# myrrix/myrrix-recommender

Measured on AMD Instinct MI355X. Metric: ALS rows solved/sec (full iteration) at k=64, higher is better.
Workload: dtype f32 storage; per-row Gramian: f16x2-split operands (22 bits), f32 accumulate; Cholesky f32

## Files before the change

myrrix-recommender_amd/csrc/als_kernels.h:

```cpp
#pragma once
#include <hip/hip_runtime.h>
#include <stdint.h>

#include <type_traits>

namespace mals {

#ifndef MALS_WAVES
#define MALS_WAVES(T, MODE) ((T) <= 4 ? 4 : ((T) == 5 ? 3 : 2))
#endif
#ifndef MALS_WAVES_H
#define MALS_WAVES_H(T, MODE) ((T) <= 2 ? 5 : ((T) <= 4 ? 3 : 2))
#endif

typedef float f32x4 __attribute__((ext_vector_type(4)));
typedef double f64x4 __attribute__((ext_vector_type(4)));

__host__ __device__ constexpr int tri(int T) { return T * (T + 1) / 2; }
__host__ __device__ constexpr int tidx(int T, int i, int j) { return i * T - (i * (i - 1)) / 2 + (j - i); }

constexpr int YMAX_SLOTS = 64;

struct WorkItem {
  int64_t begin;
// ... 1638 lines not shown
  }
  if (Gf) {
    const float f = (row < k && col < k) ? (float)s : 0.f;
    const int lr = row - 16 * i, lc = col - 16 * j;
    Gf[(t * 64 + 16 * (lr >> 2) + lc) * 4 + (lr & 3)] = f;
    if (i == j) Gf[(t * 64 + 16 * (lc >> 2) + lr) * 4 + (lc & 3)] = f;
  }
}

__global__ void gramian_ref_latch_kernel(int* state) { state[3] = (state[0] != 0 && state[1] == 0) ? 1 : 0; }

template <int T>
__global__ __launch_bounds__(256) void gramian_ref_kernel(const float* __restrict__ M, int64_t n_rows, int k, int* state,
                                                          double* __restrict__ part, double* __restrict__ Gref) {
  if (state[3] == 0) return;
  constexpr int KP = 16 * T, NE = T * T;
  __shared__ float srow[8][KP];
  __shared__ int s_last;
  const int tid = threadIdx.x;
  double acc[NE];
#pragma unroll
  for (int j = 0; j < NE; ++j) acc[j] = 0.0;
  const int64_t per = (n_rows + gridDim.x - 1) / gridDim.x;
  const int64_t r0 = per * blockIdx.x, r1 = r0 + per < n_rows ? r0 + per : n_rows;
  for (int64_t base = r0; base < r1; base += 8) {
    __syncthreads();
    for (int e = tid; e < 8 * KP; e += 256) {
      const int i = e / KP, f = e - i * KP;
      srow[i][f] = (base + i < r1 && f < k) ? M[(base + i) * k + f] : 0.f;
    }
    __syncthreads();
#pragma unroll
    for (int i = 0; i < 8; ++i) {
#pragma unroll
      for (int j = 0; j < NE; ++j) {
        const int e = tid + 256 * j, r = e / KP, c = e - r * KP;
        acc[j] += (double)__fmul_rn(srow[i][r], srow[i][c]);
      }
    }
  }
#pragma unroll
  for (int j = 0; j < NE; ++j) part[(size_t)blockIdx.x * (KP * KP) + tid + 256 * j] = acc[j];
  __threadfence();
  __syncthreads();
  if (tid == 0) s_last = atomicAdd(&state[2], 1) == (int)gridDim.x - 1;
  __syncthreads();
  if (!s_last) return;
  __threadfence();
#pragma unroll
  for (int j = 0; j < NE; ++j) {
    const int e = tid + 256 * j, r = e / KP, c = e - r * KP;
    double sum = 0.0;
    for (unsigned w = 0; w < gridDim.x; ++w) sum += part[(size_t)w * (KP * KP) + e];
    if (r < k && c < k) Gref[(int64_t)r * k + c] = sum;
  }
  __threadfence();
  __syncthreads();
  if (tid == 0) {
    state[2] = 0;
    state[1] = 1;
  }
}

template <int T>
__global__ __launch_bounds__(256, 2) void gramian_split_kernel(const float* __restrict__ M, int64_t n_rows, int k,
                                                               int64_t rows_per_slab, float* __restrict__ partial,
                                                               unsigned* __restrict__ ymax) {
  constexpr int E = T <= 4 ? 8 : 4, STEP = 4 * E;
  const int lane = threadIdx.x & 63, g = lane >> 4, c = lane & 15;
  const int64_t slab = uniform64((int64_t)blockIdx.x * 4 + (threadIdx.x >> 6));
  const int64_t r0 = slab * rows_per_slab;
  int64_t r1 = r0 + rows_per_slab;
  if (r1 > n_rows) r1 = n_rows;
  f32x4 acc[tri(T)];
#pragma unroll
  for (int t = 0; t < tri(T); ++t) acc[t] = f32x4{0.f, 0.f, 0.f, 0.f};
  int pw = 100;
  int slab_max = 0;
  const int n_slab = (int)(r1 - r0);
  const float* __restrict__ base = M + (n_slab > 0 ? r0 : 0) * k;
  const bool kfull = k == 16 * T;
  int fo[T];
#pragma unroll
  for (int v = 0; v < T; ++v) fo[v] = 16 * v + c < k ? 16 * v + c : k - 1;
  auto load_step = [&](int rl, float (&raw)[T][E]) {
    if (rl + STEP <= n_slab) {
      const char* bb = reinterpret_cast<const char*>(base);
      const unsigned o0 = 4u * (unsigned)((rl + E * g) * k + c), last = 4u * (unsigned)(fo[T - 1] - c);
      if (kfull) {
#pragma unroll
        for (int s4 = 0; s4 < E; ++s4) {
          const unsigned o = o0 + 4u * (unsigned)(s4 * k);
#pragma unroll
          for (int v = 0; v < T; ++v) raw[v][s4] = *reinterpret_cast<const float*>(bb + o + 64 * v);
        }
      } else {
#pragma unroll
        for (int s4 = 0; s4 < E; ++s4) {
          const unsigned o = o0 + 4u * (unsigned)(s4 * k);
#pragma unroll
          for (int v = 0; v < T - 1; ++v) raw[v][s4] = *reinterpret_cast<const float*>(bb + o + 64 * v);
          raw[T - 1][s4] = *reinterpret_cast<const float*>(bb + (o + last));
        }
      }
    } else {
#pragma unroll
      for (int s4 = 0; s4 < E; ++s4) {
        const int row = rl + E * g + s4;
        const unsigned o = (unsigned)((row < n_slab ? row : 0) * k);
#pragma unroll
        for (int v = 0; v < T; ++v) raw[v][s4] = base[o + (unsigned)fo[v]];
      }
    }
  };
  auto do_step = [&](int rl, float (&raw)[T][E], int reload) {
    if (rl + STEP > n_slab) {
#pragma unroll
      for (int s4 = 0; s4 < E; ++s4)
        if (!(rl + E * g + s4 < n_slab))
#pragma unroll
          for (int v = 0; v < T; ++v) raw[v][s4] = 0.f;
    }
    if (!kfull) {
      if (!(16 * (T - 1) + c < k))
#pragma unroll
        for (int s4 = 0; s4 < E; ++s4) raw[T - 1][s4] = 0.f;
    }
    float amax = 0.f;
#pragma unroll
    for (int s4 = 0; s4 < E; ++s4)
#pragma unroll
      for (int v = 0; v < T; ++v) amax = fmaxf(amax, fabsf(raw[v][s4]));
    int m = __float_as_int(amax);
    for (int off = 32; off > 0; off >>= 1) m = max(m, __shfl_xor(m, off));
    m = uniform(m);
    slab_max = max(slab_max, m);
    if (m != 0) {
      const int eb = ((m >> 23) & 255) - 126;
      const int want = 14 - eb;
      if (want < pw) {
        if (pw != 100) {
          int d2 = 2 * (want - pw);
          d2 = d2 < -120 ? -120 : d2;
          const float f = __int_as_float((d2 + 127) << 23);
#pragma unroll
          for (int t = 0; t < tri(T); ++t) acc[t] *= f;
        }
        pw = want;
      }
    }
    const int pwc = pw == 100 ? 0 : (pw < -100 ? -100 : (pw > 100 ? 100 : pw));
    const float sc = __int_as_float((pwc + 127) << 23);
    ZOp<E> zh[T], zl[T];
#pragma unroll
    for (int v = 0; v < T; ++v) {
#pragma unroll
      for (int pr = 0; pr < E / 2; ++pr) {
        const float z0 = raw[v][2 * pr] * sc, z1 = raw[v][2 * pr + 1] * sc;
        const int h01 = pk_rn16(z0, z1);
        zh[v].r[pr] = h01;
        zl[v].r[pr] = pk_rn16(residual_lo(h01, z0), residual_hi(h01, z1));
      }
    }
    __builtin_amdgcn_sched_barrier(0);
    load_step(reload, raw);
    __builtin_amdgcn_sched_barrier(0);
#pragma unroll
    for (int i = 0; i < T; ++i)
#pragma unroll
      for (int j = i; j < T; ++j) acc[tidx(T, i, j)] = mfma_h<E>(zh[i], zh[j], acc[tidx(T, i, j)]);
#pragma unroll
    for (int i = 0; i < T; ++i)
#pragma unroll
      for (int j = i; j < T; ++j) acc[tidx(T, i, j)] = mfma_h<E>(zh[i], zl[j], acc[tidx(T, i, j)]);
#pragma unroll
    for (int i = 0; i < T; ++i)
#pragma unroll
      for (int j = i; j < T; ++j) acc[tidx(T, i, j)] = mfma_h<E>(zl[i], zh[j], acc[tidx(T, i, j)]);
  };
  if constexpr (T <= 6) {
    float ra[T][E], rb[T][E];
    load_step(0, ra);
    load_step(STEP, rb);
    for (int rl = 0; rl < n_slab; rl += 2 * STEP) {
      do_step(rl, ra, rl + 2 * STEP);
      do_step(rl + STEP, rb, rl + 3 * STEP);
    }
  } else {
    float ra[T][E];
    load_step(0, ra);
    for (int rl = 0; rl < n_slab; rl += STEP) do_step(rl, ra, rl + STEP);
  }
  int d2 = pw == 100 ? 0 : -2 * pw;
  d2 = d2 < -126 ? -126 : (d2 > 126 ? 126 : d2);
  const float back = __int_as_float((d2 + 127) << 23);
  float* o = partial + slab * (int64_t)(tri(T) * 4 * 64) + lane;
#pragma unroll
  for (int t = 0; t < tri(T); ++t)
#pragma unroll
    for (int r = 0; r < 4; ++r) o[(t * 4 + r) * 64] = acc[t][r] * back;
  if (ymax) {
    __shared__ int s_max[4];
    if (lane == 0) s_max[threadIdx.x >> 6] = slab_max;
    __syncthreads();
    if (threadIdx.x == 0) {
      const unsigned m4 = (unsigned)max(max(s_max[0], s_max[1]), max(s_max[2], s_max[3]));
      unsigned* slot = ymax + (blockIdx.x & (YMAX_SLOTS - 1));
      if (m4 > __builtin_nontemporal_load(slot)) atomicMax(slot, m4);
    }
  }
}

__global__ void gramian_pack_kernel(const double* __restrict__ G, int k, int T, float* __restrict__ Gf) {
  const int e = blockIdx.x * blockDim.x + threadIdx.x;
  if (e >= tri(T) * 256) return;
  const int t = e >> 8, lane = (e >> 2) & 63, reg = e & 3;
  int i = 0, rem = t;
  while (rem >= T - i) {
    rem -= T - i;
    ++i;
  }
  const int j = i + rem;
  const int row = 16 * i + 4 * (lane >> 4) + reg, col = 16 * j + (lane & 15);
  Gf[e] = (row < k && col < k) ? (float)G[(int64_t)row * k + col] : 0.f;
}

__global__ void gather_scale_kernel(const double* __restrict__ G, int k, float sqrt_w_max, float sqrt_w_mean, double n_rows,
                                    int force_flag, const unsigned* __restrict__ ymax, float* __restrict__ out) {
  if (blockIdx.x != 0 || threadIdx.x >= 64) return;
  const int lane = threadIdx.x;
  double d = 0.0, tr = 0.0;
  for (int f = lane; f < k; f += 64) {
    const double g = G[(int64_t)f * k + f];
    d = fmax(d, g);
    tr += g;
  }
  unsigned bits = (ymax && lane < YMAX_SLOTS) ? ymax[lane] : 0u;
  static_assert(YMAX_SLOTS <= 64, "one slot per lane");
  for (int off = 32; off > 0; off >>= 1) {
    d = fmax(d, __shfl_xor(d, off));
    tr += __shfl_xor(tr, off);
    bits = max(bits, (unsigned)__shfl_xor((int)bits, off));
  }
  if (lane != 0) return;
  double ybound = sqrt(d);
  if (ymax) {
    const float ym = __uint_as_float(bits);
    if (ym > 0.f && ym < 3.0e38f && (double)ym < ybound) ybound = (double)ym;
  }
  out[3] = (float)ybound;
  const double bound = ybound * (double)sqrt_w_max;
  int e = 0;
  if (bound > 0.0 && bound < 1.0e300) {
    int eb;
    (void)frexp(bound, &eb);
    e = 14 - eb;
    e = e < -60 ? -60 : (e > 60 ? 60 : e);
  }
  out[0] = (float)ldexp(1.0, e);
  out[1] = (float)ldexp(1.0, -2 * e);
  const double typical = (double)sqrt_w_mean * sqrt(tr / ((double)k * fmax(n_rows, 1.0)));
  float ok = 1.f;
  if (typical > 0.0 && bound > 0.0 && bound / typical > 65536.0) ok = 0.f;
  if (!(bound < 1.0e300)) ok = 0.f;
  if (force_flag >= 0) ok = (float)force_flag;
  out[2] = ok;
}

__global__ void max_abs_kernel(const float* __restrict__ v, int64_t n, unsigned* __restrict__ out, double* __restrict__ sum_out) {
  float m = 0.f;
  double s = 0.0;
  for (int64_t i = (int64_t)blockIdx.x * blockDim.x + threadIdx.x; i < n; i += (int64_t)gridDim.x * blockDim.x) {
    const float a = fabsf(v[i]);
    m = fmaxf(m, a);
    s += (double)a;
  }
  for (int off = 32; off > 0; off >>= 1) {
    m = fmaxf(m, __shfl_xor(m, off));
    s += __shfl_xor(s, off);
  }
  if ((threadIdx.x & 63) == 0) {
    atomicMax(out, __float_as_uint(m));
    atomicAdd(sum_out, s);
  }
}

__global__ void col_range_kernel(const int32_t* __restrict__ col, int64_t n, int* __restrict__ out) {
  int lo = 0x7fffffff, hi = (int)0x80000000;
  for (int64_t i = (int64_t)blockIdx.x * blockDim.x + threadIdx.x; i < n; i += (int64_t)gridDim.x * blockDim.x) {
    const int c = col[i];
    lo = min(lo, c);
    hi = max(hi, c);
  }
  for (int off = 32; off > 0; off >>= 1) {
    lo = min(lo, __shfl_xor(lo, off));
    hi = max(hi, __shfl_xor(hi, off));
  }
  if ((threadIdx.x & 63) == 0) {
    atomicMin(out, lo);
    atomicMax(out + 1, hi);
  }
}

template <int T>
__global__ __launch_bounds__(256) void reconstruction_kernel(const int64_t* __restrict__ row_ptr, const int32_t* __restrict__ col,
                                                             const float* __restrict__ X, const float* __restrict__ Y, int k,
                                                             int64_t n_rows, double* __restrict__ partial_sum,
                                                             unsigned long long* __restrict__ partial_cnt) {
  const int lane = threadIdx.x & 63, g = lane >> 4, c = lane & 15;
  const int64_t wave = (int64_t)blockIdx.x * 4 + (threadIdx.x >> 6), n_waves = (int64_t)gridDim.x * 4;
  double acc = 0.0;
  unsigned long long cnt = 0;
  for (int64_t row = wave; row < n_rows; row += n_waves) {
    const int64_t b = row_ptr[row], e = row_ptr[row + 1];
    float x[T];
#pragma unroll
    for (int v = 0; v < T; ++v) x[v] = 16 * v + c < k ? X[row * k + 16 * v + c] : 0.f;
    for (int64_t s = b; s < e; s += 4) {
      const bool ok = s + g < e;
      const float* y = Y + (int64_t)col[ok ? s + g : b] * k;
      double d = 0.0;
#pragma unroll
      for (int v = 0; v < T; ++v) {
        const float yv = 16 * v + c < k ? y[16 * v + c] : 0.f;
        d += (double)__fmul_rn(x[v], yv);
      }
#pragma unroll
      for (int off = 8; off > 0; off >>= 1) d += __shfl_xor(d, off);
      if (ok && c == 0) {
        acc += fmax(0.0, 1.0 - d);
        ++cnt;
      }
    }
  }
  acc += __shfl_xor(acc, 16);
  acc += __shfl_xor(acc, 32);
  cnt += __shfl_xor(cnt, 16);
  cnt += __shfl_xor(cnt, 32);
  if (lane == 0) {
    partial_sum[wave] = acc;
    partial_cnt[wave] = cnt;
  }
}

__global__ void sample_dots_kernel(const float* __restrict__ X, const float* __restrict__ Y, const int64_t* __restrict__ users,
                                   const int64_t* __restrict__ items, int n_users, int n_items, int k, double* __restrict__ out) {
  const int e = blockIdx.x * blockDim.x + threadIdx.x;
  if (e >= n_users * n_items) return;
  const float* x = X + users[e / n_items] * (int64_t)k;
  const float* y = Y + items[e % n_items] * (int64_t)k;
  double d = 0.0;
  for (int f = 0; f < k; ++f) d += (double)__fmul_rn(x[f], y[f]);
  out[e] = d;
}

__global__ void pad_rows_kernel(const float* __restrict__ src, int64_t n, int k, int ld, float* __restrict__ dst) {
  const int q = ld >> 2;
  const int64_t n4 = n * q;
  for (int64_t e = (int64_t)blockIdx.x * blockDim.x + threadIdx.x; e < n4; e += (int64_t)gridDim.x * blockDim.x) {
    const int64_t r = e / q;
    const int f = 4 * (int)(e - r * q);
    const float* s = src + r * k + f;
    f32x4 v;
#pragma unroll
    for (int i = 0; i < 4; ++i) v[i] = f + i < k ? s[i] : 0.f;
    reinterpret_cast<f32x4*>(dst)[e] = v;
  }
}

__global__ void gather_rows_kernel(const float* __restrict__ F, const int64_t* __restrict__ idx, int n, int k,
                                   float* __restrict__ out) {
  const int e = blockIdx.x * blockDim.x + threadIdx.x;
  if (e >= n * k) return;
  out[e] = F[idx[e / k] * (int64_t)k + (e % k)];
}

}
```

myrrix-recommender_amd/csrc/mals_api.hip:

```cpp
#include "../../include/myrrix_als.h"
#include "als_kernels.h"
#include "dual_kernels.h"
#include "lds_kernels.h"
#include "host_eigen.h"
#include "host_solver.h"
#include "topn_kernels.h"
#include "mals_internal.h"
#include "hip_buffer.h"

#include <hip/hip_runtime.h>

#include <algorithm>
#include <atomic>
#include <chrono>
#include <cmath>
#include <cstdio>
#include <cstdlib>
#include <condition_variable>
#include <cstring>
#include <deque>
#include <limits>
#include <mutex>
#include <new>
#include <string>
#include <thread>
#include <type_traits>
#include <vector>

#ifndef MALS_D4
#define MALS_D4 4
#endif
using namespace mals;

namespace {

struct SideState {
  int64_t n_total = 0;
  float* F = nullptr;
  DeviceBuffer<float> F_own;
  int64_t row_offset = 0, n_local = 0, nnz = 0;
  int64_t* row_ptr = nullptr;
  int32_t* col = nullptr;
  float* val = nullptr;
  DeviceBuffer<int64_t> row_ptr_own;
  DeviceBuffer<int32_t> col_own;
  DeviceBuffer<float> val_own;
  bool has_matrix = false;
  std::vector<int64_t> h_row_ptr;
  int64_t append_rows = 0, append_nnz = 0;
  bool appending = false;
  DeviceBuffer<WorkItem> itemsA;
  int64_t nA = 0;
  int64_t nnzA = 0, nnzB = 0;
  DeviceBuffer<WorkItem> itemsB;
  int64_t nB = 0;
  DeviceBuffer<RowC> rowsC;
  int64_t nC = 0;
  DeviceBuffer<float> scratch;
  DeviceBuffer<uint8_t> refine;
  int32_t col_min = 0, col_max = -1;
  float max_abs_val = 0.f;
  float local_max_abs_val = 0.f;
  double mean_abs_val = 0.0;
  double local_mean_abs_val = 0.0;
  struct ChunkRange {
    int64_t offA = 0, nA = 0, nnzA = 0, offB = 0, nB = 0, nnzB = 0, offC = 0, nC = 0;
    int64_t offP = 0, nP = 0;
    int64_t nD[4] = {0, 0, 0, 0}, nnzD[4] = {0, 0, 0, 0}, nZ = 0;
    int64_t n_dual() const { return nD[0] + nD[1] + nD[2] + nD[3]; }
    int64_t nnz_dual() const { return nnzD[0] + nnzD[1] + nnzD[2] + nnzD[3]; }
  };
  int64_t n_dual_rows = 0;
  int64_t chunk_rows_override = -1;
  std::vector<ChunkRange> chunks;
  DeviceBuffer<double> G;
  DeviceBuffer<float> Gf;
  DeviceBuffer<uint8_t> partials;
  bool G_valid = false;
  uint64_t G_version = 0;
  DeviceBuffer<unsigned> d_ymax;
  uint64_t ymax_version = 0;
  uint64_t F_epoch = 0;
};

struct PendingEvent {
  hipEvent_t a, b;
  int kind;
  double bytes;
};

}

struct mals_handle_s {
  mals_config cfg;
  int T = 0;
  bool split_f16 = false;
  bool split3 = false;
  int dual_blocks = 0;
  DeviceBuffer<float> d_Mr;
  DeviceBuffer<float> d_Mp;
  float refine_limit = 64.f;
  bool exact_ready = false;
  DeviceBuffer<int> d_gref_state;
  DeviceBuffer<double> d_Gref;
  DeviceBuffer<double> d_gref_part;
  DeviceBuffer<unsigned long long> d_refined;
  int pad_side = -1;
  uint64_t pad_version = 0;
  uint64_t pad_epoch = 0;
  std::vector<uint8_t> pad_done;
  DeviceBuffer<char> d_eig;
  double* d_Q = nullptr;
  float* d_Qf = nullptr;
  bool rotate_f64 = false;
  bool rotate_split = false;
  int32_t* d_Bs = nullptr;
  size_t Bs_stride = 0;
  float* d_lam = nullptr;
  DeviceBuffer<unsigned> d_zbound;
  PinnedBuffer<double> h_G;
  hipEvent_t ev_G = nullptr;
  PinnedBuffer<char> eig_stage;
  bool eig_ok = false;
  double eig_gmax = 0.0;
  bool dual_pending = false;
  int dual_pending_side = -1, dual_pending_chunk = -1;
  double tl[4] = {0.0, 0.0, 0.0, 0.0};
  int dual_side = -1;
  uint64_t dual_version = 0;
  bool dual_ok = false;
  hipEvent_t ev_ready = nullptr, ev_refine = nullptr;
  bool refine_recorded = false;
  mals_iteration_fn iter_fn = nullptr;
  void* iter_user = nullptr;
  bool lds_gather = false;
  DeviceBuffer<float> d_Gperm;
  int gperm_side = -1;
  uint64_t gperm_version = 0;
  DeviceBuffer<float> d_zscale;
  int zs_side = -1;
  uint64_t zs_version = 0;
  float zs_bound = -1.f;
  double zs_mean = -1.0;
  DeviceBuffer<unsigned> d_maxabs;
  DeviceBuffer<int> d_colrange;
  int n_cu = 256;
  SideState side[2];
  hipStream_t stream = nullptr;
  hipStream_t aux[2] = {nullptr, nullptr};
  hipEvent_t ev_fork = nullptr, ev_join[2] = {nullptr, nullptr};
  bool overlap = false;
  bool forked[2] = {false, false};
  std::string err;
  DeviceBuffer<unsigned long long> d_bad;
  PinnedBuffer<unsigned long long> h_bad;
  int32_t sing_side = -1;
  int64_t sing_row = -1;
  int32_t sing_rank = 0;
  std::atomic<int> cancelled{0};
  bool timing = false;
  mals_stats stats;
  std::vector<PendingEvent> pending;
  DeviceBuffer<unsigned long long> d_trace;
  void* tn_ws = nullptr;
  void* tn_front = nullptr;
  DeviceBuffer<uint32_t> tag_bits;
  int64_t tag_bits_items = 0, n_tag_items = 0;
  const int64_t* known_ptr = nullptr;
  const int32_t* known_idx = nullptr;
  int64_t known_rows = 0;
  DeviceBuffer<int64_t> known_ptr_copy;
  DeviceBuffer<int32_t> known_idx_copy;
  DeviceBuffer<double> d_sd;
  DeviceBuffer<int64_t> d_sd_idx;
  DeviceBuffer<int64_t> d_idx;
  DeviceBuffer<float> d_rows;
};

namespace {

int fail(mals_handle h, int code, const std::string& msg) {
  if (h) h->err = msg;
  return code;
}

#define HIPCHK(h, call)                                                                     \
  do {                                                                                      \
    hipError_t _e = (call);                                                                 \
    if (_e != hipSuccess) {                                                                 \
      const int _code = (_e == hipErrorOutOfMemory) ? MALS_OOM : MALS_HIP_ERROR;            \
      return fail(h, _code, std::string(#call) + ": " + hipGetErrorString(_e));             \
    }                                                                                       \
  } while (0)

#define CHECK_SIDE(h, side)                                                  \
  do {                                                                       \
    if (!(h)) return MALS_INVALID_ARG;                                       \
    if ((side) != MALS_SIDE_X && (side) != MALS_SIDE_Y)                      \
      return fail(h, MALS_INVALID_ARG, "side must be MALS_SIDE_X or _Y");    \
  } while (0)

int use_device(mals_handle h) {
  HIPCHK(h, hipSetDevice(h->cfg.device));
  return MALS_OK;
}

void clear_known_items(mals_handle h) {
  h->known_ptr_copy.reset();
  h->known_idx_copy.reset();
  h->known_ptr = nullptr;
  h->known_idx = nullptr;
  h->known_rows = 0;
}

void free_matrix(SideState& s) {
  s.row_ptr_own.reset();
  s.col_own.reset();
  s.val_own.reset();
  s.row_ptr = nullptr;
  s.col = nullptr;
  s.val = nullptr;
  s.has_matrix = false;
  s.itemsA.reset();
  s.itemsB.reset();
  s.rowsC.reset();
  s.scratch.reset();
  s.refine.reset();
  s.nA = s.nB = s.nC = 0;
  s.nnzA = s.nnzB = 0;
  s.chunks.clear();
  s.h_row_ptr.clear();
  s.h_row_ptr.shrink_to_fit();
}

int alloc_matrix(mals_handle h, SideState& s) {
  HIPCHK(h, s.row_ptr_own.alloc((size_t)(s.n_local + 1)));
  HIPCHK(h, s.col_own.alloc((size_t)std::max<int64_t>(s.nnz, 1)));
  HIPCHK(h, s.val_own.alloc((size_t)std::max<int64_t>(s.nnz, 1)));
  s.row_ptr = s.row_ptr_own.get();
  s.col = s.col_own.get();
  s.val = s.val_own.get();
  return MALS_OK;
}

int64_t slot_floats(int T) { return (int64_t)(tri(T) * 4 + T) * 64; }

int build_work_lists(mals_handle h, SideState& s) {
  s.max_abs_val = 0.f;
  s.mean_abs_val = 0.0;
  s.local_mean_abs_val = 0.0;
  s.n_dual_rows = 0;
  if (s.nnz > 0) {
    HIPCHK(h, hipMemsetAsync(h->d_maxabs.get(), 0, 4 * sizeof(unsigned), h->stream));
    const unsigned blocks = (unsigned)std::min<int64_t>(4096, (s.nnz + 255) / 256);
    hipLaunchKernelGGL(max_abs_kernel, dim3(blocks), dim3(256), 0, h->stream, s.val, s.nnz, h->d_maxabs.get(),
                       reinterpret_cast<double*>(h->d_maxabs.get() + 2));
    HIPCHK(h, hipGetLastError());
    unsigned raw[4];
    HIPCHK(h, hipMemcpyAsync(raw, h->d_maxabs.get(), sizeof(raw), hipMemcpyDeviceToHost, h->stream));
    HIPCHK(h, hipStreamSynchronize(h->stream));
    std::memcpy(&s.max_abs_val, &raw[0], sizeof(float));
    double sum = 0.0;
    std::memcpy(&sum, &raw[2], sizeof(double));
    s.mean_abs_val = sum / (double)s.nnz;
    s.local_mean_abs_val = s.mean_abs_val;
  }
  s.local_max_abs_val = s.max_abs_val;
  s.col_min = 0;
  s.col_max = -1;
  if (s.nnz > 0) {
    const int init[2] = {std::numeric_limits<int>::max(), std::numeric_limits<int>::min()};
    HIPCHK(h, hipMemcpyAsync(h->d_colrange.get(), init, sizeof(init), hipMemcpyHostToDevice, h->stream));
    const unsigned blocks = (unsigned)std::min<int64_t>(4096, (s.nnz + 255) / 256);
    hipLaunchKernelGGL(col_range_kernel, dim3(blocks), dim3(256), 0, h->stream, s.col, s.nnz, h->d_colrange.get());
    HIPCHK(h, hipGetLastError());
    int range[2];
    HIPCHK(h, hipMemcpyAsync(range, h->d_colrange.get(), sizeof(range), hipMemcpyDeviceToHost, h->stream));
    HIPCHK(h, hipStreamSynchronize(h->stream));
    s.col_min = range[0];
    s.col_max = range[1];
    if (s.col_min < 0) return fail(h, MALS_INVALID_ARG, "negative column index");
  }
  const int64_t n = s.n_local;
  const int seg = h->cfg.segment_nnz;
  const int64_t want_chunk = s.chunk_rows_override >= 0 ? s.chunk_rows_override : h->cfg.chunk_rows;
  const int64_t chunk_rows = want_chunk > 0 ? want_chunk : std::max<int64_t>(n, 1);
  const int n_chunks = (int)std::max<int64_t>(1, (n + chunk_rows - 1) / chunk_rows);
  const std::vector<int64_t>& rp = s.h_row_ptr;
  std::vector<WorkItem> order;
  std::vector<WorkItem> segs;
  std::vector<RowC> rowsC, groups;
  order.reserve((size_t)n);
  int64_t slot = 0;
  s.chunks.assign((size_t)n_chunks, SideState::ChunkRange());
  std::vector<int64_t> count((size_t)seg + 2);
  for (int c = 0; c < n_chunks; ++c) {
    const int64_t r0 = std::min(n, c * chunk_rows), r1 = std::min(n, (c + 1) * chunk_rows);
    SideState::ChunkRange& cr = s.chunks[(size_t)c];
    cr.offA = (int64_t)order.size();
    cr.offB = (int64_t)segs.size();
    cr.offC = (int64_t)rowsC.size();
    std::fill(count.begin(), count.end(), 0);
    const int64_t dual_len = 16 * (int64_t)h->dual_blocks;
    int64_t n_short = 0, n_direct = 0, n_empty = 0;
    for (int64_t r = r0; r < r1; ++r) {
      const int64_t len = rp[r + 1] - rp[r];
      if (len < 0) return fail(h, MALS_INVALID_ARG, "row_ptr must be non-decreasing");
      if (len <= seg) {
        ++count[(size_t)(seg - len)];
        ++n_short;
        if (len == 0) {
          ++n_empty;
        } else if (len <= dual_len) {
          const int cls = (int)((len - 1) >> 4);
          ++cr.nD[cls];
          cr.nnzD[cls] += len;
        } else {
          ++n_direct;
          cr.nnzA += len;
        }
      } else {
        cr.nnzB += len;
      }
    }
    int64_t seg_b = seg;
    {
      const int64_t want_segments = (int64_t)h->n_cu * 4;
      const int64_t lo = std::min<int64_t>(512, seg);
      seg_b = std::max<int64_t>(lo, std::min<int64_t>(seg, (cr.nnzB + want_segments - 1) / want_segments));
      seg_b = (seg_b + 31) & ~(int64_t)31;
      if (seg_b > seg) seg_b = seg;
    }
    int64_t acc = cr.offA;
    for (size_t b = 0; b < count.size(); ++b) {
      const int64_t cnt = count[b];
      count[b] = acc;
      acc += cnt;
    }
    order.resize((size_t)(cr.offA + n_short));
    for (int64_t r = r0; r < r1; ++r) {
      const int64_t len = rp[r + 1] - rp[r];
      if (len <= seg) {
        WorkItem& w = order[(size_t)count[(size_t)(seg - len)]++];
        w.begin = rp[r];
        w.len = (int32_t)len;
        w.id = (int32_t)r;
      } else {
        const int64_t nseg = (len + seg_b - 1) / seg_b;
        int64_t per = (len + nseg - 1) / nseg;
        per = (per + 3) & ~(int64_t)3;
        RowC rc;
        rc.first_slot = slot;
        rc.row = (int32_t)r;
        rc.nseg = 0;
        rc.stride = 1;
        rc.pad_ = 0;
        for (int64_t b = 0; b < len; b += per) {
          if (slot >= std::numeric_limits<int32_t>::max()) return fail(h, MALS_INVALID_ARG, "too many row segments");
          WorkItem sg;
          sg.begin = rp[r] + b;
          sg.len = (int32_t)std::min(per, len - b);
          sg.id = (int32_t)slot++;
          segs.push_back(sg);
          ++rc.nseg;
        }
        if (rc.nseg > FINISH_GROUP) {
          const int32_t grp_len = FINISH_GROUP;
          for (int32_t g0 = 0; g0 < rc.nseg; g0 += grp_len) {
            RowC grp;
            grp.first_slot = rc.first_slot + g0;
            grp.row = (int32_t)r;
            grp.nseg = std::min<int32_t>(grp_len, rc.nseg - g0);
            grp.stride = 1;
            grp.pad_ = 0;
            groups.push_back(grp);
          }
          rc.nseg = (rc.nseg + grp_len - 1) / grp_len;
          rc.stride = grp_len;
        }
        rowsC.push_back(rc);
      }
    }
    const int64_t n_dual = cr.n_dual();
    if (n_empty > 0 && n_dual > 0) {
      auto first = order.begin() + (size_t)(cr.offA + n_direct);
      std::rotate(first, first + (size_t)n_dual, first + (size_t)n_dual + 1);
    }
    cr.nA = n_direct + (n_empty > 0 ? 1 : 0);
    cr.nZ = n_empty > 0 ? n_empty - 1 : 0;
    s.n_dual_rows += n_dual;
    cr.nB = (int64_t)segs.size() - cr.offB;
    cr.nC = (int64_t)rowsC.size() - cr.offC;
    cr.offP = (int64_t)rowsC.size();
    cr.nP = (int64_t)groups.size();
    rowsC.insert(rowsC.end(), groups.begin(), groups.end());
    groups.clear();
    std::stable_sort(segs.begin() + cr.offB, segs.end(), [](const WorkItem& a, const WorkItem& b) { return a.len > b.len; });
    s.nnzA += cr.nnzA;
    s.nnzB += cr.nnzB;
  }
  s.nA = (int64_t)order.size();
  s.nB = (int64_t)segs.size();
  s.nC = (int64_t)rowsC.size();
  if (std::getenv("MALS_DEBUG_LISTS")) {
    int64_t nd[4] = {0, 0, 0, 0}, ed[4] = {0, 0, 0, 0}, na = 0, nz = 0, n_long = 0;
    for (const SideState::ChunkRange& cr : s.chunks) {
      n_long += cr.nC;
      for (int c = 0; c < 4; ++c) {
        nd[c] += cr.nD[c];
        ed[c] += cr.nnzD[c];
      }
      na += cr.nA;
      nz += cr.nZ;
    }
    std::fprintf(stderr, "[lists] rows %lld: direct %lld (%lld entries), dual 1-16: %lld (%lld) 17-32: %lld (%lld) 33-48: %lld (%lld) 49-64: %lld (%lld), "
                         "zero-filled %lld, segments %lld of %lld long rows (%lld entries)\n",
                 (long long)n, (long long)na, (long long)s.nnzA, (long long)nd[0], (long long)ed[0], (long long)nd[1], (long long)ed[1], (long long)nd[2],
                 (long long)ed[2], (long long)nd[3], (long long)ed[3], (long long)nz, (long long)s.nB, (long long)n_long, (long long)s.nnzB);
  }
  if (s.nA) {
    HIPCHK(h, s.itemsA.alloc(order.size()));
    HIPCHK(h, hipMemcpy(s.itemsA.get(), order.data(), sizeof(WorkItem) * order.size(), hipMemcpyHostToDevice));
  }
  if (s.nB) {
    HIPCHK(h, s.itemsB.alloc(segs.size()));
    HIPCHK(h, hipMemcpy(s.itemsB.get(), segs.data(), sizeof(WorkItem) * segs.size(), hipMemcpyHostToDevice));
    HIPCHK(h, s.rowsC.alloc(rowsC.size()));
    HIPCHK(h, hipMemcpy(s.rowsC.get(), rowsC.data(), sizeof(RowC) * rowsC.size(), hipMemcpyHostToDevice));
    HIPCHK(h, s.scratch.alloc((size_t)(slot * slot_floats(h->T))));
  }
  return MALS_OK;
}

int validate_matrix(mals_handle h, int side) {
  SideState& s = h->side[side];
  if (s.h_row_ptr.size() != (size_t)s.n_local + 1 || s.h_row_ptr[0] != 0 || s.h_row_ptr[(size_t)s.n_local] != s.nnz)
    return fail(h, MALS_INVALID_ARG, "row_ptr must have n_rows_local+1 entries, start at 0 and end at nnz");
  return MALS_OK;
}

int validate_columns(mals_handle h, int side) {
  const SideState& s = h->side[side];
  const SideState& o = h->side[1 - side];
  if (s.nnz > 0 && o.n_total > 0 && (int64_t)s.col_max >= o.n_total)
    return fail(h, MALS_INVALID_ARG, "column index outside the opposite side's factor replica");
  return MALS_OK;
}

int begin_timed(mals_handle h, int kind, double bytes, PendingEvent& pe) {
  pe.kind = kind;
  pe.bytes = bytes;
  pe.a = pe.b = nullptr;
  if (!h->timing) return MALS_OK;
  HIPCHK(h, hipEventCreate(&pe.a));
  HIPCHK(h, hipEventCreate(&pe.b));
  HIPCHK(h, hipEventRecord(pe.a, h->stream));
  return MALS_OK;
}
int end_timed(mals_handle h, PendingEvent& pe) {
  if (!h->timing) return MALS_OK;
  HIPCHK(h, hipEventRecord(pe.b, h->stream));
  h->pending.push_back(pe);
  return MALS_OK;
}
int drain_events(mals_handle h) {
  for (PendingEvent& pe : h->pending) {
    HIPCHK(h, hipEventSynchronize(pe.b));
    float ms = 0.f;
    HIPCHK(h, hipEventElapsedTime(&ms, pe.a, pe.b));
    mals_stats& st = h->stats;
    switch (pe.kind) {
      case 0: st.rows_ms += ms; st.rows_launches += 1; st.rows_bytes += pe.bytes; break;
      case 1: st.segments_ms += ms; st.segments_launches += 1; st.segments_bytes += pe.bytes; break;
      case 2: st.finish_ms += ms; st.finish_launches += 1; st.finish_bytes += pe.bytes; break;
      case 4: st.dual_ms += ms; st.dual_launches += 1; st.dual_bytes += pe.bytes; break;
      case 5: st.rotate_ms += ms; st.rotate_launches += 1; st.rotate_bytes += pe.bytes; break;
      default: st.gramian_ms += ms; st.gramian_launches += 1; st.gramian_bytes += pe.bytes; break;
    }
    (void)hipEventDestroy(pe.a);
    (void)hipEventDestroy(pe.b);
  }
  h->pending.clear();
  return MALS_OK;
}

constexpr int64_t GRAMIAN_SPLIT_MIN_ROWS = 262144;
inline int64_t gramian_slab_rows(int64_t n_rows) {
  static const int64_t forced = std::getenv("MALS_GRAMIAN_SLAB_ROWS") ? std::atoll(std::getenv("MALS_GRAMIAN_SLAB_ROWS")) : 0;
  if (forced > 0) return forced;
  int64_t slab = 512;
  while (slab < 2048 && n_rows / (2 * slab) / 4 >= 1024) slab *= 2;
  return slab;
}

template <int T>
int launch_gramian_T(mals_handle h, SideState& s, const float* M, int64_t n_rows, double* G_out, float* Gf_out, unsigned* ymax) {
  const int k = h->cfg.features;
  const int elems = tri(T) * 256;
  static const bool force_f64 = std::getenv("MALS_GRAMIAN_F64") != nullptr;
  if (n_rows >= GRAMIAN_SPLIT_MIN_ROWS && !force_f64) {
    const int64_t slab_rows = gramian_slab_rows(n_rows);
    int64_t n_slabs = (n_rows + slab_rows - 1) / slab_rows;
    n_slabs = (n_slabs + 3) & ~(int64_t)3;
    constexpr int GROUPS = 64;
    const size_t slab_bytes = sizeof(float) * (size_t)n_slabs * tri(T) * 256;
    const size_t bytes = slab_bytes + sizeof(double) * (size_t)GROUPS * tri(T) * 256;
    if (s.partials.capacity() < bytes) HIPCHK(h, s.partials.alloc(bytes));
    float* pf = reinterpret_cast<float*>(s.partials.get());
    double* pd = reinterpret_cast<double*>(s.partials.get() + slab_bytes);
    hipLaunchKernelGGL((gramian_split_kernel<T>), dim3((unsigned)(n_slabs / 4)), dim3(256), 0, h->stream, M, n_rows, k,
                       slab_rows, pf, ymax);
    hipLaunchKernelGGL(gramian_reduce_slabs_kernel, dim3((unsigned)((elems + 255) / 256), GROUPS), dim3(256), 0, h->stream, pf, n_slabs,
                       elems, GROUPS, pd);
    hipLaunchKernelGGL((gramian_finalize_kernel<T, false>), dim3(elems / 64), dim3(256), 0, h->stream, pd, (int64_t)GROUPS, k, G_out, Gf_out);
    HIPCHK(h, hipGetLastError());
    return MALS_OK;
  }
  int64_t n_waves = std::min<int64_t>(1024, std::max<int64_t>(1, (n_rows + 63) / 64));
  n_waves = (n_waves + 3) & ~(int64_t)3;
  int64_t rows_per_wave = (n_rows + n_waves - 1) / n_waves;
  rows_per_wave = std::max<int64_t>(4, (rows_per_wave + 3) & ~(int64_t)3);
  const size_t bytes = sizeof(double) * (size_t)n_waves * tri(T) * 256;
  if (s.partials.capacity() < bytes) HIPCHK(h, s.partials.alloc(bytes));
  double* partials = reinterpret_cast<double*>(s.partials.get());
  if (ymax) HIPCHK(h, hipMemsetAsync(ymax, 0x7f, sizeof(unsigned), h->stream));
  hipLaunchKernelGGL((gramian_partial_kernel<T>), dim3((unsigned)(n_waves / 4)), dim3(256), 0, h->stream, M, n_rows, k,
                     rows_per_wave, partials);
  hipLaunchKernelGGL((gramian_finalize_kernel<T, true, 16>), dim3(elems / 16), dim3(256), 0, h->stream, partials, n_waves,
                     k, G_out, Gf_out);
  HIPCHK(h, hipGetLastError());
  return MALS_OK;
}

int launch_gramian(mals_handle h, SideState& s, const float* M, int64_t n_rows, double* G_out, float* Gf_out, unsigned* ymax = nullptr) {
  switch (h->T) {
    case 1: return launch_gramian_T<1>(h, s, M, n_rows, G_out, Gf_out, ymax);
    case 2: return launch_gramian_T<2>(h, s, M, n_rows, G_out, Gf_out, ymax);
    case 3: return launch_gramian_T<3>(h, s, M, n_rows, G_out, Gf_out, ymax);
    case 4: return launch_gramian_T<4>(h, s, M, n_rows, G_out, Gf_out, ymax);
    case 5: return launch_gramian_T<5>(h, s, M, n_rows, G_out, Gf_out, ymax);
    case 6: return launch_gramian_T<6>(h, s, M, n_rows, G_out, Gf_out, ymax);
    case 7: return launch_gramian_T<7>(h, s, M, n_rows, G_out, Gf_out, ymax);
    case 8: return launch_gramian_T<8>(h, s, M, n_rows, G_out, Gf_out, ymax);
  }
  return fail(h, MALS_INVALID_ARG, "unsupported feature count");
}

template <typename K>
int persistent_grid(mals_handle h, K kernel, int64_t n_work, unsigned* grid) {
  int per_cu = 0;
  HIPCHK(h, hipOccupancyMaxActiveBlocksPerMultiprocessor(&per_cu, kernel, 256, 0));
  if (per_cu < 1) per_cu = 1;
  per_cu *= 16;
  if (const char* e = std::getenv("MALS_BLOCKS_PER_CU")) per_cu = std::max(1, std::atoi(e));
  const int64_t cap = (int64_t)h->n_cu * per_cu;
  *grid = (unsigned)std::max<int64_t>(1, std::min<int64_t>((n_work + 3) / 4, cap));
  return MALS_OK;
}

enum { LISTS_ROWS = 1, LISTS_DUAL_ROWS = 2, LISTS_LONG = 4, LISTS_OWN = LISTS_ROWS | LISTS_LONG };

template <typename K, typename KF>
int launch_persistent(mals_handle h, K kernel, KF fallback, const SolveParams& p, int kind, double bytes) {
  PendingEvent pe;
  unsigned grid = 1;
  if (int rc = persistent_grid(h, kernel, p.n_work, &grid)) return rc;
  if (int rc = begin_timed(h, kind, bytes, pe)) return rc;
  hipLaunchKernelGGL(kernel, dim3(grid), dim3(256), 0, h->stream, p);
  if constexpr (!std::is_same<KF, std::nullptr_t>::value) {
    SolveParams pf = p;
    pf.flags |= 8;
    if (int rc = persistent_grid(h, fallback, p.n_work, &grid)) return rc;
    grid = std::min<unsigned>(grid, (unsigned)h->n_cu * 8u);
    hipLaunchKernelGGL(fallback, dim3(grid), dim3(256), 0, h->stream, pf);
  }
  return end_timed(h, pe);
}

template <typename KA, typename KB, typename KFA, typename KFB, typename KC, typename KP>
int launch_lists(mals_handle h, SideState& s, SolveParams p, int chunk, int which, KA rows_kernel, KB segments_kernel, KFA rows_fallback,
                 KFB segments_fallback, KC finish_kernel, KP prereduce_kernel) {
  const double per = 4.0 * p.k + 8.0;
  const SideState::ChunkRange& cr = s.chunks[(size_t)chunk];
  PendingEvent pe;
  const bool own = which & LISTS_ROWS, longs = which & LISTS_LONG, dual_rows_too = which & LISTS_DUAL_ROWS;
  if (longs && cr.nB) {
    p.n_work = cr.nB;
    p.items = s.itemsB.get() + cr.offB;
    if (int rc = launch_persistent(h, segments_kernel, segments_fallback, p, 1, (double)cr.nnzB * per)) return rc;
  }
  if (own && cr.nA) {
    p.n_work = cr.nA;
    p.items = s.itemsA.get() + cr.offA;
    if (int rc = launch_persistent(h, rows_kernel, rows_fallback, p, 0, (double)cr.nnzA * per + (double)cr.nA * per)) return rc;
  }
  if (dual_rows_too && cr.n_dual()) {
    p.n_work = cr.n_dual();
    p.items = s.itemsA.get() + cr.offA + cr.nA;
    if (int rc = launch_persistent(h, rows_kernel, rows_fallback, p, 0, (double)cr.nnz_dual() * per + (double)cr.n_dual() * per)) return rc;
  }
  if (longs && cr.nC) {
    if (int rc = begin_timed(h, 2, (double)cr.nC * per, pe)) return rc;
    if (cr.nP) {
      p.n_work = cr.nP;
      p.rowsC = s.rowsC.get() + cr.offP;
      hipLaunchKernelGGL(prereduce_kernel, dim3((unsigned)((cr.nP + 3) / 4)), dim3(256), 0, h->stream, p);
    }
    p.n_work = cr.nC;
    p.rowsC = s.rowsC.get() + cr.offC;
    hipLaunchKernelGGL(finish_kernel, dim3((unsigned)((cr.nC + 3) / 4)), dim3(256), 0, h->stream, p);
    if (int rc = end_timed(h, pe)) return rc;
  }
  if (own && cr.nZ) {
    hipLaunchKernelGGL(zero_rows_kernel, dim3((unsigned)((cr.nZ + 31) / 32)), dim3(256), 0, h->stream,
                       s.itemsA.get() + cr.offA + cr.nA + cr.n_dual(), cr.nZ, p.k, p.out);
  }
  HIPCHK(h, hipGetLastError());
  return MALS_OK;
}

template <typename K, typename KF>
int launch_persistent_lds(mals_handle h, K kernel, KF fallback, const SolveParams& p, int kind, double bytes) {
  PendingEvent pe;
  int per_cu = 8 * 16;
  if (const char* e = std::getenv("MALS_BLOCKS_PER_CU")) per_cu = std::max(1, std::atoi(e)) * 4;
  unsigned grid = (unsigned)std::max<int64_t>(1, std::min<int64_t>(p.n_work, (int64_t)h->n_cu * per_cu));
  if (int rc = begin_timed(h, kind, bytes, pe)) return rc;
  hipLaunchKernelGGL(kernel, dim3(grid), dim3(64), 0, h->stream, p);
  SolveParams pf = p;
  pf.flags |= 8;
  if (int rc = persistent_grid(h, fallback, p.n_work, &grid)) return rc;
  grid = std::min<unsigned>(grid, (unsigned)h->n_cu * 8u);
  hipLaunchKernelGGL(fallback, dim3(grid), dim3(256), 0, h->stream, pf);
  return end_timed(h, pe);
}

int launch_lists_lds(mals_handle h, SideState& s, SolveParams p, int chunk, int which) {
  constexpr int T = 8, D = 2;
  const double per = 4.0 * p.k + 8.0;
  const SideState::ChunkRange& cr = s.chunks[(size_t)chunk];
  PendingEvent pe;
  const bool own = which & LISTS_ROWS, longs = which & LISTS_LONG, dual_rows_too = which & LISTS_DUAL_ROWS;
  if (longs && cr.nB) {
    p.n_work = cr.nB;
    p.items = s.itemsB.get() + cr.offB;
    if (int rc = launch_persistent_lds(h, als_lds_kernel_h<1>, als_persistent_kernel<T, D, 1, true>, p, 1, (double)cr.nnzB * per)) return rc;
  }
  if (own && cr.nA) {
    p.n_work = cr.nA;
    p.items = s.itemsA.get() + cr.offA;
    if (int rc = launch_persistent_lds(h, als_lds_kernel_h<0>, als_persistent_kernel<T, D, 0, true>, p, 0, (double)cr.nnzA * per + (double)cr.nA * per)) return rc;
  }
  if (dual_rows_too && cr.n_dual()) {
    p.n_work = cr.n_dual();
    p.items = s.itemsA.get() + cr.offA + cr.nA;
    if (int rc = launch_persistent_lds(h, als_lds_kernel_h<0>, als_persistent_kernel<T, D, 0, true>, p, 0,
                                       (double)cr.nnz_dual() * per + (double)cr.n_dual() * per)) return rc;
  }
  if (longs && cr.nC) {
    if (int rc = begin_timed(h, 2, (double)cr.nC * per, pe)) return rc;
    if (cr.nP) {
      p.n_work = cr.nP;
      p.rowsC = s.rowsC.get() + cr.offP;
      hipLaunchKernelGGL(als_prereduce_kernel<T>, dim3((unsigned)((cr.nP + 3) / 4)), dim3(256), 0, h->stream, p);
    }
    p.n_work = cr.nC;
    p.rowsC = s.rowsC.get() + cr.offC;
    hipLaunchKernelGGL((als_finish_kernel<T, true>), dim3((unsigned)((cr.nC + 3) / 4)), dim3(256), 0, h->stream, p);
    SolveParams pf = p;
    pf.flags |= 8;
    hipLaunchKernelGGL((als_finish_kernel<T, false>), dim3((unsigned)((cr.nC + 3) / 4)), dim3(256), 0, h->stream, pf);
    if (int rc = end_timed(h, pe)) return rc;
  }
  if (own && cr.nZ) {
    hipLaunchKernelGGL(zero_rows_kernel, dim3((unsigned)((cr.nZ + 31) / 32)), dim3(256), 0, h->stream,
                       s.itemsA.get() + cr.offA + cr.nA + cr.n_dual(), cr.nZ, p.k, p.out);
  }
  HIPCHK(h, hipGetLastError());
  return MALS_OK;
}

template <int T, int D, bool FULL>
int launch_solve_TF(mals_handle h, SideState& s, const SolveParams& p, int chunk, int which) {
  if constexpr (T == 8 && FULL) {
    if (h->split_f16 && h->lds_gather && p.Gperm) return launch_lists_lds(h, s, p, chunk, which);
  }
  if constexpr (T == 4) {
    if (h->split3)
      return launch_lists(h, s, p, chunk, which, als_persistent_kernel_h<T, 0, FULL, 3>, als_persistent_kernel_h<T, 1, FULL, 3>,
                          als_persistent_kernel<T, D, 0, FULL>, als_persistent_kernel<T, D, 1, FULL>, als_finish_kernel<T>,
                          als_prereduce_kernel<T>);
  }
  if (h->split_f16)
    return launch_lists(h, s, p, chunk, which, als_persistent_kernel_h<T, 0, FULL>, als_persistent_kernel_h<T, 1, FULL>,
                        als_persistent_kernel<T, D, 0, FULL>, als_persistent_kernel<T, D, 1, FULL>, als_finish_kernel<T>,
                        als_prereduce_kernel<T>);
  return launch_lists(h, s, p, chunk, which, als_persistent_kernel<T, D, 0, FULL>, als_persistent_kernel<T, D, 1, FULL>,
                      nullptr, nullptr, als_finish_kernel<T>, als_prereduce_kernel<T>);
}

template <int T, int D>
int launch_solve_T(mals_handle h, SideState& s, const SolveParams& p, int chunk, int which) {
  return p.k == 16 * T ? launch_solve_TF<T, D, true>(h, s, p, chunk, which) : launch_solve_TF<T, D, false>(h, s, p, chunk, which);
}

int launch_solve(mals_handle h, SideState& s, const SolveParams& p, int chunk, int which) {
  switch (h->T) {
    case 1: return launch_solve_T<1, 4>(h, s, p, chunk, which);
    case 2: return launch_solve_T<2, 4>(h, s, p, chunk, which);
    case 3: return launch_solve_T<3, 4>(h, s, p, chunk, which);
    case 4: return launch_solve_T<4, MALS_D4>(h, s, p, chunk, which);
    case 5: return launch_solve_T<5, 2>(h, s, p, chunk, which);
    case 6: return launch_solve_T<6, 2>(h, s, p, chunk, which);
    case 7: return launch_solve_T<7, 2>(h, s, p, chunk, which);
    case 8: return launch_solve_T<8, 2>(h, s, p, chunk, which);
  }
  return fail(h, MALS_INVALID_ARG, "unsupported feature count");
}

template <int T>
int launch_refine_T(mals_handle h, const RefineParams& q) {
// ... 1779 lines not shown
```

Before: 136.3 million.

## Cut long rows at column bands and order segments by band for cache reuse

Adds a setup pass that finds, for each long row, where its column indices cross fixed column-band edges sized to about 64 MiB of factor rows. Long rows are split at those edges when the columns ascend, and segments are sorted by band and then by length. The aim is for concurrently running waves to read the same slice of the other-side factor matrix, so it stays in cache instead of streaming from HBM. It only engages when the factor table exceeds 256 MiB, and it adds setup kernels plus host sorting.

New measurement: 139.6 million, median of 6. 2.4% higher.

```diff
diff --git a/myrrix-recommender_amd/csrc/als_kernels.h b/myrrix-recommender_amd/csrc/als_kernels.h
--- a/myrrix-recommender_amd/csrc/als_kernels.h
+++ b/myrrix-recommender_amd/csrc/als_kernels.h
@@ -1964,6 +1964,47 @@
   }
 }
 
+constexpr int BAND_UNIT = 4096;
+__global__ __launch_bounds__(256) void band_order_kernel(const int64_t* __restrict__ row_ptr, const int32_t* __restrict__ col,
+                                                         const int32_t* __restrict__ rows, const int2* __restrict__ units, int64_t n_units,
+                                                         int32_t* __restrict__ descent) {
+  const int lane = threadIdx.x & 63;
+  const int64_t wave = (int64_t)blockIdx.x * 4 + (threadIdx.x >> 6), n_waves = (int64_t)gridDim.x * 4;
+  for (int64_t u = wave; u < n_units; u += n_waves) {
+    const int2 un = units[u];
+    const int r = rows[un.x];
+    const int64_t b0 = row_ptr[r], len = row_ptr[r + 1] - b0;
+    const int64_t j0 = (int64_t)un.y * BAND_UNIT, j1 = min(len - 1, j0 + BAND_UNIT);
+    bool bad = false;
+    for (int64_t j = j0 + lane; j < j1; j += 64) bad |= col[b0 + j] > col[b0 + j + 1];
+    if (__ballot(bad) != 0 && lane == 0) descent[un.x] = 1;
+  }
+}
+__global__ __launch_bounds__(256) void band_cuts_kernel(const int64_t* __restrict__ row_ptr, const int32_t* __restrict__ col,
+                                                        const int32_t* __restrict__ rows, const int32_t* __restrict__ descent, int64_t n_rows,
+                                                        int64_t col0, int64_t band_cols, int n_bands, int32_t* __restrict__ out) {
+  const int lane = threadIdx.x & 63;
+  const int64_t wave = (int64_t)blockIdx.x * 4 + (threadIdx.x >> 6), n_waves = (int64_t)gridDim.x * 4;
+  for (int64_t i = wave; i < n_rows; i += n_waves) {
+    const int r = rows[i];
+    const int64_t b0 = row_ptr[r], len = row_ptr[r + 1] - b0;
+    int32_t* o = out + i * (n_bands + 1);
+    for (int b = lane; b <= n_bands; b += 64) {
+      int64_t lo = b == n_bands ? len : 0;
+      if (b > 0 && b < n_bands) {
+        const int64_t edge = col0 + (int64_t)b * band_cols;
+        int64_t hi = len;
+        while (lo < hi) {
+          const int64_t mid = (lo + hi) >> 1;
+          if ((int64_t)col[b0 + mid] < edge) lo = mid + 1;
+          else hi = mid;
+        }
+      }
+      o[b] = (b == 0 && descent[i] != 0) ? -1 : (int32_t)lo;
+    }
+  }
+}
+
 template <int T>
 __global__ __launch_bounds__(256) void reconstruction_kernel(const int64_t* __restrict__ row_ptr, const int32_t* __restrict__ col,
                                                              const float* __restrict__ X, const float* __restrict__ Y, int k,
diff --git a/myrrix-recommender_amd/csrc/band_cuts.h b/myrrix-recommender_amd/csrc/band_cuts.h
--- /dev/null
+++ b/myrrix-recommender_amd/csrc/band_cuts.h
@@ -0,0 +1,64 @@
+#pragma once
+
+#include <algorithm>
+#include <cstdint>
+#include <vector>
+
+namespace mals {
+
+struct BandPiece {
+  int64_t off;
+  int32_t len;
+  int32_t band;
+};
+
+inline void equal_pieces(int64_t off, int64_t len, int64_t seg_b, std::vector<BandPiece>& out) {
+  const int64_t nseg = (len + seg_b - 1) / seg_b;
+  int64_t per = (len + nseg - 1) / nseg;
+  per = (per + 3) & ~(int64_t)3;
+  for (int64_t b = 0; b < len; b += per) out.push_back(BandPiece{off + b, (int32_t)std::min(per, len - b), 0});
+}
+
+inline bool band_pieces(int64_t len, const int32_t* cuts, int n_bands, int64_t seg_b, int64_t min_piece, std::vector<BandPiece>& out) {
+  const size_t first = out.size();
+  bool ascending = cuts != nullptr && n_bands >= 1 && cuts[0] == 0 && cuts[n_bands] == len;
+  for (int b = 0; ascending && b < n_bands; ++b) ascending = cuts[b] <= cuts[b + 1];
+  bool banded = ascending && n_bands >= 2 && len >= 2 * min_piece;
+  if (banded) {
+    auto edge = [&](int b) -> int64_t { return b == n_bands ? len : (int64_t)(cuts[b] & ~3); };
+    int64_t start = 0;
+    std::vector<int64_t> ends;
+    for (int b = 1; b <= n_bands; ++b) {
+      const int64_t e = edge(b);
+      if (e - start >= min_piece) {
+        ends.push_back(e);
+        start = e;
+      }
+    }
+    if (start < len) {
+      if (ends.empty()) ends.push_back(len);
+      else ends.back() = len;
+    }
+    banded = ends.size() >= 2;
+    if (banded) {
+      start = 0;
+      for (const int64_t e : ends) {
+        equal_pieces(start, e - start, seg_b, out);
+        start = e;
+      }
+    }
+  }
+  if (!banded) equal_pieces(0, len, seg_b, out);
+  int b = 0;
+  for (size_t i = first; i < out.size(); ++i) {
+    if (!ascending) {
+      out[i].band = -1;
+      continue;
+    }
+    while (b + 1 < n_bands && (int64_t)(cuts[b + 1] & ~3) <= out[i].off) ++b;
+    out[i].band = b;
+  }
+  return banded;
+}
+
+}
diff --git a/myrrix-recommender_amd/csrc/mals_api.hip b/myrrix-recommender_amd/csrc/mals_api.hip
--- a/myrrix-recommender_amd/csrc/mals_api.hip
+++ b/myrrix-recommender_amd/csrc/mals_api.hip
@@ -7,6 +7,7 @@
 #include "topn_kernels.h"
 #include "mals_internal.h"
 #include "hip_buffer.h"
+#include "band_cuts.h"
 
 #include <hip/hip_runtime.h>
 
@@ -245,6 +246,66 @@
 
 int64_t slot_floats(int T) { return (int64_t)(tri(T) * 4 + T) * 64; }
 
+constexpr int64_t BAND_BYTES = 64ll << 20;
+constexpr int64_t BAND_MIN_TABLE = 256ll << 20;
+constexpr int64_t BAND_MIN_PIECE = 2048;
+constexpr int BAND_MAX_DEFAULT = 256;
+constexpr int MAX_BANDS = 4096;
+
+int band_cut_table(mals_handle h, const SideState& s, int& n_bands, int64_t& band_cols, std::vector<int32_t>& cut_tab) {
+  n_bands = 0;
+  band_cols = 0;
+  cut_tab.clear();
+  int64_t band_bytes = BAND_BYTES;
+  bool forced = false;
+  if (const char* e = std::getenv("MALS_BAND_BYTES")) {
+    band_bytes = std::atoll(e);
+    forced = true;
+  }
+  const int k = h->cfg.features;
+  const int64_t row_bytes = 4 * (int64_t)(k % 16 == 0 ? k : 16 * h->T);
+  const int64_t n_cols = (int64_t)s.col_max - s.col_min + 1;
+  if (band_bytes <= 0 || s.nnz == 0 || n_cols <= 1 || (!forced && n_cols * row_bytes <= BAND_MIN_TABLE)) return MALS_OK;
+  band_cols = std::max<int64_t>(1, band_bytes / row_bytes);
+  band_cols = std::max<int64_t>(band_cols, (n_cols + MAX_BANDS - 1) / MAX_BANDS);
+  const int nb = (int)((n_cols + band_cols - 1) / band_cols);
+  if (nb < 2 || (!forced && nb > BAND_MAX_DEFAULT)) return MALS_OK;
+  const int seg = h->cfg.segment_nnz;
+  const std::vector<int64_t>& rp = s.h_row_ptr;
+  std::vector<int32_t> rows;
+  std::vector<int2> units;
+  for (int64_t r = 0; r < s.n_local; ++r) {
+    const int64_t len = rp[r + 1] - rp[r];
+    if (len <= seg) continue;
+    if (len > std::numeric_limits<int32_t>::max()) return MALS_OK;
+    for (int64_t u = 0; u * BAND_UNIT < len - 1; ++u) units.push_back(int2{(int)rows.size(), (int)u});
+    rows.push_back((int32_t)r);
+  }
+  if (rows.empty()) return MALS_OK;
+  const int64_t n_rows = (int64_t)rows.size();
+  DeviceBuffer<int32_t> d_rows, d_descent, d_cuts;
+  DeviceBuffer<int2> d_units;
+  HIPCHK(h, d_rows.alloc(rows.size()));
+  HIPCHK(h, d_descent.alloc(rows.size()));
+  HIPCHK(h, d_units.alloc(units.size()));
+  HIPCHK(h, d_cuts.alloc((size_t)n_rows * (size_t)(nb + 1)));
+  HIPCHK(h, hipMemcpyAsync(d_rows.get(), rows.data(), sizeof(int32_t) * rows.size(), hipMemcpyHostToDevice, h->stream));
+  HIPCHK(h, hipMemcpyAsync(d_units.get(), units.data(), sizeof(int2) * units.size(), hipMemcpyHostToDevice, h->stream));
+  HIPCHK(h, hipMemsetAsync(d_descent.get(), 0, sizeof(int32_t) * rows.size(), h->stream));
+  const int64_t max_blocks = (int64_t)h->n_cu * 32;
+  hipLaunchKernelGGL(band_order_kernel, dim3((unsigned)std::min<int64_t>(max_blocks, ((int64_t)units.size() + 3) / 4)), dim3(256), 0, h->stream,
+                     s.row_ptr, s.col, d_rows.get(), d_units.get(), (int64_t)units.size(), d_descent.get());
+  HIPCHK(h, hipGetLastError());
+  hipLaunchKernelGGL(band_cuts_kernel, dim3((unsigned)std::min<int64_t>(max_blocks, (n_rows + 3) / 4)), dim3(256), 0, h->stream, s.row_ptr,
+                     s.col, d_rows.get(), d_descent.get(), n_rows, (int64_t)s.col_min, band_cols, nb, d_cuts.get());
+  HIPCHK(h, hipGetLastError());
+  cut_tab.resize((size_t)n_rows * (size_t)(nb + 1));
+  HIPCHK(h, hipMemcpyAsync(cut_tab.data(), d_cuts.get(), sizeof(int32_t) * cut_tab.size(), hipMemcpyDeviceToHost, h->stream));
+  HIPCHK(h, hipStreamSynchronize(h->stream));
+  n_bands = nb;
+  return MALS_OK;
+}
+
 int build_work_lists(mals_handle h, SideState& s) {
   s.max_abs_val = 0.f;
   s.mean_abs_val = 0.0;
@@ -287,6 +348,14 @@
   const int64_t chunk_rows = want_chunk > 0 ? want_chunk : std::max<int64_t>(n, 1);
   const int n_chunks = (int)std::max<int64_t>(1, (n + chunk_rows - 1) / chunk_rows);
   const std::vector<int64_t>& rp = s.h_row_ptr;
+  int n_bands = 0;
+  int64_t band_cols = 0;
+  std::vector<int32_t> cut_tab;
+  if (int rc = band_cut_table(h, s, n_bands, band_cols, cut_tab)) return rc;
+  int64_t n_long_rows = 0, n_banded_rows = 0;
+  std::vector<BandPiece> pieces;
+  std::vector<int32_t> seg_band;
+  std::vector<int64_t> seg_order;
   std::vector<WorkItem> order;
   std::vector<WorkItem> segs;
   std::vector<RowC> rowsC, groups;
@@ -346,22 +415,24 @@
         w.len = (int32_t)len;
         w.id = (int32_t)r;
       } else {
-        const int64_t nseg = (len + seg_b - 1) / seg_b;
-        int64_t per = (len + nseg - 1) / nseg;
-        per = (per + 3) & ~(int64_t)3;
+        pieces.clear();
+        const int32_t* cuts = n_bands ? cut_tab.data() + (size_t)n_long_rows * (size_t)(n_bands + 1) : nullptr;
+        n_banded_rows += band_pieces(len, cuts, n_bands, seg_b, BAND_MIN_PIECE, pieces) ? 1 : 0;
+        ++n_long_rows;
         RowC rc;
         rc.first_slot = slot;
         rc.row = (int32_t)r;
         rc.nseg = 0;
         rc.stride = 1;
         rc.pad_ = 0;
-        for (int64_t b = 0; b < len; b += per) {
+        for (const BandPiece& pc : pieces) {
           if (slot >= std::numeric_limits<int32_t>::max()) return fail(h, MALS_INVALID_ARG, "too many row segments");
           WorkItem sg;
-          sg.begin = rp[r] + b;
-          sg.len = (int32_t)std::min(per, len - b);
+          sg.begin = rp[r] + pc.off;
+          sg.len = pc.len;
           sg.id = (int32_t)slot++;
           segs.push_back(sg);
+          seg_band.push_back(pc.band);
           ++rc.nseg;
         }
         if (rc.nseg > FINISH_GROUP) {
@@ -395,7 +466,22 @@
     cr.nP = (int64_t)groups.size();
     rowsC.insert(rowsC.end(), groups.begin(), groups.end());
     groups.clear();
-    std::stable_sort(segs.begin() + cr.offB, segs.end(), [](const WorkItem& a, const WorkItem& b) { return a.len > b.len; });
+    {
+      const size_t b0 = (size_t)cr.offB, nb = segs.size() - b0;
+      seg_order.resize(nb);
+      for (size_t i = 0; i < nb; ++i) seg_order[i] = (int64_t)(b0 + i);
+      std::stable_sort(seg_order.begin(), seg_order.end(), [&](int64_t a, int64_t b) {
+        return seg_band[(size_t)a] != seg_band[(size_t)b] ? seg_band[(size_t)a] < seg_band[(size_t)b] : segs[(size_t)a].len > segs[(size_t)b].len;
+      });
+      std::vector<WorkItem> sorted(nb);
+      std::vector<int32_t> sorted_band(nb);
+      for (size_t i = 0; i < nb; ++i) {
+        sorted[i] = segs[(size_t)seg_order[i]];
+        sorted_band[i] = seg_band[(size_t)seg_order[i]];
+      }
+      std::copy(sorted.begin(), sorted.end(), segs.begin() + (int64_t)b0);
+      std::copy(sorted_band.begin(), sorted_band.end(), seg_band.begin() + (int64_t)b0);
+    }
     s.nnzA += cr.nnzA;
     s.nnzB += cr.nnzB;
   }
@@ -417,6 +503,16 @@
                          "zero-filled %lld, segments %lld of %lld long rows (%lld entries)\n",
                  (long long)n, (long long)na, (long long)s.nnzA, (long long)nd[0], (long long)ed[0], (long long)nd[1], (long long)ed[1], (long long)nd[2],
                  (long long)ed[2], (long long)nd[3], (long long)ed[3], (long long)nz, (long long)s.nB, (long long)n_long, (long long)s.nnzB);
+    if (n_bands) {
+      std::vector<int64_t> per_band((size_t)n_bands + 1, 0);
+      for (const int32_t b : seg_band) ++per_band[(size_t)(b + 1)];
+      const int64_t mx = *std::max_element(per_band.begin() + 1, per_band.end());
+      const int64_t mn = *std::min_element(per_band.begin() + 1, per_band.end());
+      std::fprintf(stderr, "[bands] %d bands of %lld columns; %lld of %lld long rows cut at bands; %lld segments of rows whose columns do "
+                           "not ascend; segments per band %lld..%lld, mean %.0f\n",
+                   n_bands, (long long)band_cols, (long long)n_banded_rows, (long long)n_long_rows, (long long)per_band[0], (long long)mn,
+                   (long long)mx, (double)(s.nB - per_band[0]) / n_bands);
+    }
   }
   if (s.nA) {
     HIPCHK(h, s.itemsA.alloc(order.size()));
```
